# harskish/fluctus

Hardware: AMD Instinct MI355X
Metric: Mrays/s (primary+shadow) at 1080p, 8 bounces (higher is better)
Workload: dtype f32; 1 GPU; kitchen-proc (procedural stand-in for Country Kitchen OBJ), 1920x1080, 8 bounces, env-map MIS under night.hdr, separate material queues; width=1920, height=1080, max_bounces=8, triangles=495648, bvh=sbvh, bvh_nodes=342315, num_tasks_per_gpu=16777216, num_tasks_whole_job=16777216, scaling_mode=weak: --num-tasks paths in flight per rank, wavefronts_per_gpu=1, fused_logic_materials=True, fused_bsdf_set=1, ext_order=2, refill_extend=8208, overlap=2, regroup=1

## Files before the change

### fluctus_amd/csrc/api.hip

```cpp
#include "flx_ctx.h"
#include <cstring>
#include <cstdlib>

thread_local std::string flxd::g_create_error;

static uint32_t localPixels(const flx_ctx *c)
{
    uint32_t npix = c->params.width * c->params.height;
    if (npix <= c->fr.rank) return 1;
    return (npix - c->fr.rank + c->fr.nranks - 1) / c->fr.nranks;
}

static int allocMoments(flx_ctx *c)
{
    freeAll(c->momAllocs);
    c->fr.moments = nullptr;
    if (!c->moments || !c->fr.localPixels) return 0;
    const size_t n = (size_t)c->fr.localPixels * 4;
    HIPCHK(c, dalloc(c, c->momAllocs, &c->fr.moments, n) ? hipErrorOutOfMemory : hipSuccess);
    HIPCHK(c, hipMemsetAsync(c->fr.moments, 0, n * 4, c->stream));
    return 0;
}
static int allocAov(flx_ctx *c)
{
// ... 85 lines not shown
        if ((e = hipStreamCreateWithPriority(&c->stream2, hipStreamNonBlocking, pSecond)) != hipSuccess) return fail("hipStreamCreate", e);
    }
    if ((e = hipEventCreateWithFlags(&c->evPreExt, hipEventDisableTiming)) != hipSuccess || (e = hipEventCreateWithFlags(&c->evShadow, hipEventDisableTiming)) != hipSuccess ||
        (e = hipEventCreateWithFlags(&c->evPostLogic, hipEventDisableTiming)) != hipSuccess) return fail("hipEventCreate", e);
    const size_t N = num_tasks;
    c->st.numTasks = num_tasks;
    for (int r = 0; r < S_NUM_REC; r++) {
        if (dalloc(c, c->fixedAllocs, &c->st.rec[r], N)) return fail("hipMalloc(state)", hipErrorOutOfMemory);
        (void)hipMemsetAsync(c->st.rec[r], 0, N * sizeof(float4), c->stream);
    }
    if (dalloc(c, c->fixedAllocs, &c->st.phase, N) || dalloc(c, c->fixedAllocs, &c->mkStats, 4)) return fail("hipMalloc(state)", hipErrorOutOfMemory);
    (void)hipMemsetAsync(c->st.phase, 0, N * 4, c->stream); (void)hipMemsetAsync(c->mkStats, 0, 16, c->stream);
    if (dalloc(c, c->fixedAllocs, &c->st.blocked, N) || dalloc(c, c->fixedAllocs, &c->st.pickProb, N) || dalloc(c, c->fixedAllocs, &c->st.firstDiffuse, N))
        return fail("hipMalloc(state)", hipErrorOutOfMemory);
    (void)hipMemsetAsync(c->st.blocked, 0, N * 4, c->stream); (void)hipMemsetAsync(c->st.pickProb, 0, N * 4, c->stream); (void)hipMemsetAsync(c->st.firstDiffuse, 0, N * 4, c->stream);
    for (int q = 0; q < FLX_NUM_QUEUES; q++) {
        if (dalloc(c, c->fixedAllocs, &c->qs.q[q], N)) return fail("hipMalloc(queue)", hipErrorOutOfMemory);
        (void)hipMemsetAsync(c->qs.q[q], 0, N * 4, c->stream);
    }
    if (dalloc(c, c->fixedAllocs, &c->qs.counters, 8) || dalloc(c, c->fixedAllocs, &c->qs.cursors, FLX_NUM_BLOCK_CURSORS * FLX_CURSOR_STRIDE)) return fail("hipMalloc(counters)", hipErrorOutOfMemory);
    (void)hipMemsetAsync(c->qs.counters, 0, 32, c->stream);
    (void)hipMemsetAsync(c->qs.cursors, 0, 4 * FLX_NUM_BLOCK_CURSORS * FLX_CURSOR_STRIDE, c->stream);
    const size_t auxStride = logic_aux_stride(num_tasks);
    if (dalloc(c, c->fixedAllocs, &c->member, N) || dalloc(c, c->fixedAllocs, &c->blockCounts, (size_t)7 * auxStride) || dalloc(c, c->fixedAllocs, &c->blockOffsets, (size_t)7 * auxStride))
        return fail("hipMalloc(logic aux)", hipErrorOutOfMemory);
    if (dalloc(c, c->fixedAllocs, &c->logicError, 1)) return fail("hipMalloc(logic error flag)", hipErrorOutOfMemory);
    (void)hipMemsetAsync(c->logicError, 0, 4, c->stream);
    (void)hipMemsetAsync(c->blockCounts, 0, (size_t)7 * auxStride * 4, c->stream);
    (void)hipMemsetAsync(c->blockOffsets, 0, (size_t)7 * auxStride * 4, c->stream);
    { hipDeviceProp_t prop; if (hipGetDeviceProperties(&prop, device) == hipSuccess && prop.multiProcessorCount > 0) c->numCUs = prop.multiProcessorCount; }
    if (dalloc(c, c->fixedAllocs, &c->stats, FLX_NUM_TRACE_STATS)) return fail("hipMalloc(stats)", hipErrorOutOfMemory);
    (void)hipMemsetAsync(c->stats, 0, FLX_NUM_TRACE_STATS * 8, c->stream);
#ifdef FLX_LAB_RSTATS
    flxd::g_lab_rstats = c->stats;
#endif
    c->splitCapA = ((num_tasks / 2 / shadow_split_lists()) + 64u) & ~63u; c->splitCapB = ((num_tasks / 8 / shadow_split_lists()) + 64u) & ~63u;
    if (dalloc(c, c->fixedAllocs, &c->totals, 8)) return fail("hipMalloc(totals)", hipErrorOutOfMemory);
    (void)hipMemsetAsync(c->totals, 0, 64, c->stream);
    if (dalloc(c, c->fixedAllocs, &c->fr.currPixelIdx, 1)) return fail("hipMalloc(cursor)", hipErrorOutOfMemory);
    (void)hipMemsetAsync(c->fr.currPixelIdx, 0, 4, c->stream);
    c->fr.rank = 0; c->fr.nranks = 1; c->fr.localPixels = 0;
    if ((e = hipHostMalloc((void **)&c->pinned, sizeof(flx_queue_counters) * c->pinnedSlots)) != hipSuccess) return fail("hipHostMalloc", e);
    if ((e = hipHostMalloc((void **)&c->pinnedIdx, sizeof(uint32_t) * c->pinnedSlots)) != hipSuccess) return fail("hipHostMalloc", e);
    if ((e = hipHostMalloc((void **)&c->pinnedMk, 16 * c->pinnedSlots)) != hipSuccess) return fail("hipHostMalloc", e);
    {
        float4 *rgba; float2 *rec; float *pdf;
        if (dalloc(c, c->envAllocs, &rgba, 1) || dalloc(c, c->envAllocs, &rec, 1) || dalloc(c, c->envAllocs, &pdf, 1))
            return fail("hipMalloc(env)", hipErrorOutOfMemory);
        const float one = 1.0f; const float2 rec1 = make_float2(1.0f, 0.0f );
        (void)hipMemsetAsync(rgba, 0, 16, c->stream);
        (void)hipMemcpy(rec, &rec1, 8, hipMemcpyHostToDevice); (void)hipMemcpy(pdf, &one, 4, hipMemcpyHostToDevice);
        c->sc.envRGBA = rgba; c->sc.aliasRec = rec; c->sc.pdfTable = pdf; c->sc.envW = c->sc.envH = 1;
// ... 231 lines not shown
```

### fluctus_amd/csrc/api_wavefront.hip

```cpp
#include "flx_ctx.h"

struct Step { bool launchDeferred, commitRaw; int next; };
static Step transition(int ph, Call call)
{
    const bool deferred = ph == PH_DEFER_LOGIC || ph == PH_DEFER_LOGIC_RAYGEN;
    const bool chain = deferred || ph == PH_CHAIN || ph == PH_CHAIN_EXT;
    switch (call) {
    case CALL_LOGIC:     return {deferred, false, PH_IDLE};
    case CALL_RAYGEN:    if (ph == PH_DEFER_LOGIC) return {false, false, PH_DEFER_LOGIC_RAYGEN};
                         return {deferred, false, chain ? PH_CHAIN : PH_IDLE};
    case CALL_MATERIALS: if (deferred) return {false, false, PH_CHAIN};
                         return {false, true, chain ? PH_CHAIN : PH_IDLE};
    case CALL_EXTEND:    return {deferred, true, chain ? PH_CHAIN_EXT : PH_EXT};
    case CALL_SHADOW:    return {deferred, false, PH_IDLE};
    case CALL_QUIET:     return {deferred, false, deferred ? PH_CHAIN : ph};
    case CALL_NEUTRAL:   return {deferred, false, PH_IDLE};
    case CALL_PEEK:      return {deferred, true, deferred ? PH_CHAIN : ph};
    case CALL_OBSERVE:   return {deferred, true, PH_IDLE};
    }
    return {deferred, true, PH_IDLE};
}
void flxd::flushExt(flx_ctx *c) { if (c->qs.extPend) { launch_bump_extension(c->stream, c->qs.counters, c->qs.extPend); c->qs.extPend = 0; } }
static void flushExtIfPending(flx_ctx *c, uint32_t bits) { if (c->qs.extPend & bits) flushExt(c); }
static int runRaygen(flx_ctx *c, int appendExt = 1, bool alreadyDone = false, bool prepared = false)
// ... 12 lines not shown
    HIPCHK(c, hipSetDevice(c->device));
    launch_materialise(c->stream, c->st, c->sc, c->params, (uint32_t)c->numCUs);
    LAUNCHED(c);
    return 0;
}
static int extOrderFor(const flx_ctx *c, int fused, int raygenFirst) { return !fused ? 0 : (c->extOrder == 2 && (!raygenFirst || !c->raygenQueueEmpty)) ? 1 : c->extOrder; }
int flxd::fuseSetNow(const flx_ctx *c) { return c->params.wfSeparateQueues ? c->fuseSet : 31; }
static int runLogic(flx_ctx *c, int first, int fused, int raygenFirst)
{
    const int raw = (c->rawHits && fused != 0 && raygenFirst && !first) ? 1 : 0;
    if (!raw && materialise(c)) return 1;
    c->rawHits = false;
    flushExt(c);
#ifdef FLX_LAB_NOJOIN
    if (c->labIter >= 2) HIPCHK(c, hipStreamWaitEvent(c->stream, c->evLab[c->labIter & 1u], 0));
#endif
    const int order = extOrderFor(c, fused, raygenFirst);
    const int regen = (raw && c->regenOpt && c->lookback && logic_can_regenerate() && c->raygenQueueEmpty && c->fr.localPixels > 0 && c->numTasks <= (1u << 26)) ? 1 : 0;
    c->regenDone = regen != 0;
    if (regen) c->regenUsed = true;
    const int prep = (raw && !regen && c->prepOpt && c->raygenQueueEmpty && c->fr.localPixels > 0) ? 1 : 0;
    c->prepDone = prep != 0;
    if (++c->logicEpoch == 0u) c->logicEpoch = 1u;
    { ScopedTimer t(c, fused ? FLX_K_LOGIC_FUSED : FLX_K_LOGIC); launch_logic(c->stream, c->st, c->qs, c->sc, c->fr, c->params, c->member, c->blockCounts, c->blockOffsets, first, fused, raygenFirst, order, raw,
                                                                                c->lookback, c->logicEpoch, regen ? 1 : (prep ? 2 : 0), order == 2 ? 0 : 1, c->logicError, c->regroup,
                                                                                (!fused && c->ml.state.litWavefront()) ? &c->ml.t : nullptr); }
    LAUNCHED(c);
    c->matQueuesEmpty = false; c->raygenQueueEmpty = false;
    if (c->overlap == 2) HIPCHK(c, hipEventRecord(c->evPostLogic, c->stream));
    return 0;
}
static uint32_t materialBits(const flx_ctx *c)
{
    return c->params.wfSeparateQueues ? ((1u << FLX_Q_DIFFUSE) | (1u << FLX_Q_GLOSSY) | (1u << FLX_Q_GGX_REFL) | (1u << FLX_Q_GGX_REFR) | (1u << FLX_Q_DELTA)) : (1u << FLX_Q_DIFFUSE);
}
int flxd::enter(flx_ctx *c, Call call)
{
    const Step st = transition(c->phase, call);
    if (st.launchDeferred) {
        const bool withRaygen = c->phase == PH_DEFER_LOGIC_RAYGEN;
        c->phase = PH_CHAIN;
        HIPCHK(c, hipSetDevice(c->device));
        if (runLogic(c, c->pendFirst, 0, 0)) return 1;
        if (withRaygen && runRaygen(c)) return 1;
    }
    if (st.commitRaw && materialise(c)) return 1;
    c->phase = st.next;
    return 0;
// ... 141 lines not shown
```

### fluctus_amd/csrc/flx_ctx.h

```cpp
#pragma once
#include "flx_launch.h"
#include "flx_feature_state.h"
#include "../../include/fluctus_hip.h"
#include <string>
#include <vector>
#include <utility>
#include <rccl/rccl.h>

using namespace flxd;

namespace flxd {
struct PendingCounters { void *user; int slot; };
struct PendingEvent { int kernel; hipEvent_t a, b; };
inline void freeAll(std::vector<void *> &v) { for (void *p : v) (void)hipFree(p); v.clear(); }

enum Phase { PH_IDLE = 0, PH_DEFER_LOGIC = 1, PH_DEFER_LOGIC_RAYGEN = 2, PH_CHAIN = 3, PH_CHAIN_EXT = 4, PH_EXT = 5 };
enum Call {
    CALL_LOGIC, CALL_RAYGEN, CALL_MATERIALS, CALL_EXTEND, CALL_SHADOW,
    CALL_QUIET,
    CALL_NEUTRAL,
    CALL_PEEK,
    CALL_OBSERVE
};
}
// ... 6 lines not shown
#ifdef FLX_LAB_NOJOIN
    hipEvent_t evLab[2] = {nullptr, nullptr}; uint32_t labIter = 0; uint32_t *labCounters = nullptr;
#endif
    int phase = 0;
    int overlap = 2;
    int overlapOpt = -1;
    uint32_t *spill2 = nullptr;
    int fuse = 1;
    int extOrder = 0;
    int fuseSet = 1;
    int regroup = 0, regroupAuto = 0, regroupOpt = -1;
    int pendFirst = 0;
    bool matQueuesEmpty = false;
    bool raygenQueueEmpty = false;
    uint32_t numTasks = 0;
    std::string err;
    State st {};
    Queues qs {};
    Scene sc {};
    Frame fr {};
    flx_render_params params {};
    bool haveParams = false;
    uint32_t hostPixelIdx = 0;
    uint8_t *member = nullptr; uint32_t *blockCounts = nullptr, *blockOffsets = nullptr;
    unsigned long long *lookback = nullptr; uint32_t logicEpoch = 0; uint32_t *logicError = nullptr; int regenOpt = 0; bool regenDone = false; bool regenUsed = false; int prepOpt = 1; bool prepDone = false;
    uint32_t *spill = nullptr;
    unsigned long long *stats = nullptr;
    unsigned long long *totals = nullptr;
    uint32_t *mkStats = nullptr;
    uint32_t *pinnedMk = nullptr; std::vector<std::pair<void *, int>> pendingMk; int nextMkSlot = 0;
    bool statsOn = false;
    int xcdRemap = 0;
    int shadowTree = 4, extendTree = 4;
    int refillExt = 16 | (32 << 8), refillShadow = 0;
    int refillShadowOpt = -1;
    int shadowSplit = 0;
    uint32_t splitParity = 0;
    uint32_t splitLimit = 0;
    uint32_t *splitCounts = nullptr; uint4 *splitRecA = nullptr, *splitRecB = nullptr; uint32_t splitCapA = 0, splitCapB = 0;
    bool rawHits = false;
    bool cursorDirty[2] = {false, false};

    uint32_t wideInfo[8] = {0, 0, 0, 0, 0, 0, 0, 0};
    RefitTables rf;
    bool wideOK = false;
    uint32_t spillLevels = 0;
    int eagerBump = 0;
// ... 104 lines not shown
```

### fluctus_amd/csrc/flx_launch.h

```cpp
#pragma once
#include "flx_device.h"
#include <vector>

namespace flx { struct ad_params; struct rp_view; struct rp_params; }

namespace flxd {
struct RefitTables {
    uint32_t ntris = 0, nidx = 0, nmat = 0, nwtri = 0, nwleaf = 0;
    uint32_t *blevel = nullptr, *wlevel = nullptr;
    std::vector<uint32_t> blevelStart, wlevelStart;
    uint32_t *wtriOff = nullptr, *wleafOff = nullptr;
    float4 *wexact = nullptr;
    uint32_t *valid = nullptr;
    void *stage = nullptr;
    double *costSlab = nullptr;
    uint32_t *triStamp = nullptr, *bStamp = nullptr, *wStamp = nullptr, *lStamp = nullptr;
    size_t stampWords = 0;
    uint32_t epoch = 0;
    uint32_t *stageIdx = nullptr;
};
void launch_refit_validate(hipStream_t, const void *, const uint32_t *, uint32_t, const Scene &, const RefitTables &, uint32_t *);
void launch_refit(hipStream_t, const void *, const uint32_t *, uint32_t, const Scene &, const RefitTables &);
struct ObjectTables {
    uint32_t nobjects = 0, members = 0;
// ... 20 lines not shown
    *p0 = ld3(t[0]); *p1 = ld3(t[3]); *p2 = ld3(t[6]);
}
__device__ __forceinline__ int ml_material(const Scene &sc, uint32_t tri) { return sc.tris[tri].matId; }
template <bool MESH> struct MeshArg { static constexpr bool on = false; __device__ MeshLights get() const { return MeshLights(); } };
template <> struct MeshArg<true> { static constexpr bool on = true; MeshLights t; __device__ MeshLights get() const { return t; } };
uint32_t mesh_light_runs(uint32_t n);
void launch_mesh_light_build(hipStream_t, const Scene &, const MeshLights &);
void launch_mesh_light_probe(hipStream_t, const Scene &, const MeshLights &, const float *, uint32_t, uint32_t *, float *);
uint32_t pose_blocks(uint32_t members);
void launch_pose(hipStream_t, const ObjectTables &, uint32_t count);
void launch_object_of_triangle(hipStream_t, const ObjectTables &, uint32_t *objectOfTri);
void launch_block_scan(hipStream_t, uint32_t *blockCounts, uint32_t nb, uint32_t *total);
size_t tree_cost_slab_doubles(const RefitTables &);
double *launch_tree_cost(hipStream_t, const Scene &, const RefitTables &, double *);
void launch_extend(hipStream_t, const State &, const Queues &, const Scene &, const flx_render_params &, uint32_t *, unsigned long long *, int);
void launch_shadow(hipStream_t, const State &, const Queues &, const Scene &, const flx_render_params &, uint32_t *, unsigned long long *, int);
void launch_extend4(hipStream_t, const State &, const Queues &, const Scene &, const flx_render_params &, uint32_t *, unsigned long long *);
void launch_shadow4(hipStream_t, const State &, const Queues &, const Scene &, const flx_render_params &, uint32_t *, unsigned long long *);
void launch_shadow4_split(hipStream_t, const State &, const Queues &, const Scene &, const flx_render_params &, uint32_t *, uint32_t *, uint32_t, uint4 *, uint32_t, uint4 *, uint32_t, int, int, uint32_t);
uint32_t shadow_split_lists(); uint32_t shadow_split_count_words();
void launch_extend4r(hipStream_t, const State &, const Queues &, const Scene &, const flx_render_params &, uint32_t *, uint32_t, int, uint32_t *);
void launch_shadow4r(hipStream_t, const State &, const Queues &, const Scene &, const flx_render_params &, uint32_t *, uint32_t, int, uint32_t *);
void launch_logic(hipStream_t, const State &, const Queues &, const Scene &, const Frame &, const flx_render_params &, uint8_t *, uint32_t *, uint32_t *, int, int, int, int, int,
                  unsigned long long *, uint32_t, int, int, uint32_t *, int, const MeshLights *);
void launch_env_nee_table(hipStream_t, const Scene &, float4 *, uint32_t);
int logic_can_regenerate();
uint32_t logic_lookback_words(uint32_t numTasks);
void launch_materialise(hipStream_t, const State &, const Scene &, const flx_render_params &, uint32_t);
void launch_materials(hipStream_t, const State &, const Queues &, const Scene &, uint32_t);
void launch_materials_after_fused(hipStream_t, const State &, const Queues &, const Scene &, uint32_t, int);
uint32_t fused_queue_mask(int);
uint32_t logic_aux_stride(uint32_t);
void launch_reset(hipStream_t, const State &, const Queues &, const Frame &, const flx_render_params &);
void launch_raygen(hipStream_t, const State &, const Queues &, const Frame &, const flx_render_params &, int, int);
void launch_postprocess(hipStream_t, const Frame &, const flx_render_params &);
void launch_state_export(hipStream_t, const State &, float *, float);
void launch_state_import(hipStream_t, const State &, const float *);
void launch_math_probe(hipStream_t, int, const float *, const float *, uint32_t, uint32_t *);
void launch_mk_reset(hipStream_t, const State &, const Frame &, const flx_render_params &);
void launch_mk_raygen(hipStream_t, const State &, const flx_render_params &, const uint32_t *, uint32_t);
void launch_mk_next_vertex(hipStream_t, const State &, const Scene &, const Frame &, const flx_render_params &, uint32_t *, uint32_t *, const uint32_t *, uint32_t, const MeshLights *);
void launch_mk_sample_bsdf(hipStream_t, const State &, const Scene &, const Frame &, const flx_render_params &, uint32_t *, uint32_t *, const uint32_t *, uint32_t, const MeshLights *);
void launch_mk_splat(hipStream_t, const State &, const Frame &, const flx_render_params &, uint32_t *, int, const uint32_t *, uint32_t);
uint32_t adaptive_blocks(uint32_t);
void launch_adaptive_update(hipStream_t, const float4 *, int, int, const ad_params &, uint8_t *, uint32_t *, uint32_t *, uint32_t *);
void launch_end_iteration(hipStream_t, uint32_t *, unsigned long long *, uint32_t *, uint32_t, uint32_t, uint32_t *);
void launch_bump_extension(hipStream_t, uint32_t *, uint32_t);
void launch_deinterleave(hipStream_t, const float *, float *, uint32_t, uint32_t, uint32_t);
struct DnGuided; struct DnVg;
template <class F> void launch_denoise(hipStream_t, const Frame &, float4 *, float4 *, float4 *, float2 *, float *, int, int, int, float, float, float,
                                       float, const flx_render_params &);
void launch_gbuffer(hipStream_t, const Scene &, const flx_render_params &, uint32_t *, uint32_t, int, float4 *, uint32_t, uint32_t *, const uint32_t *);
void launch_reproject(hipStream_t, const rp_view &, const rp_params &, const float4 *, const float4 *, const float4 *, const float4 *, float4 *, float4 *);
void launch_reproject_motion(hipStream_t, const rp_view &, const rp_params &, const float4 *, const float4 *, const float4 *, const float4 *, float4 *, float4 *,
                             const uint32_t *, const uint32_t *, const float4 *, uint32_t);
// ... 5 lines not shown
```

### fluctus_amd/csrc/logic.hip

```cpp
#include "flx_bsdf.h"
#include "flx_trace.h"
#include "flx_denoise.h"
#include "flx_launch.h"
#include "flx_splat.h"
#include "flx_light.h"

namespace flxd {

#ifndef LOGIC_BLOCK
#define LOGIC_BLOCK 256
#endif
__host__ __device__ constexpr bool fuse_inlines_list(int fuse, uint32_t ml)
{
    return ml == 1u ? (fuse & USE_DIFFUSE) != 0 : ml == 2u ? (fuse & USE_GLOSSY) != 0 : ml == 3u ? (fuse & USE_GGX_REFL) != 0
         : ml == 4u ? (fuse & USE_GGX_REFR) != 0 : ml == 5u ? (fuse & USE_DELTA) != 0 : false;
}
#define NUM_LISTS 7

#ifndef LOGIC_FULL_STORES
#define LOGIC_FULL_STORES 1
#endif
#ifndef LOGIC_REGROUP
#define LOGIC_REGROUP 1
#endif
#ifndef LOGIC_LAZY_HITN
#define LOGIC_LAZY_HITN 1
#endif
#ifndef LOGIC_REGROUP_MIN_BLOCKS
#define LOGIC_REGROUP_MIN_BLOCKS 5
#endif

struct LogicAux {
    uint8_t *member;
    uint32_t *blockCounts;
    uint32_t *blockOffsets;
    uint32_t numBlocks;
    uint32_t stride;
    unsigned long long *lookback;
    uint32_t epoch;
    uint32_t regen;
    uint32_t appendExt;
    uint32_t *error;
};

#define LB_VALUE(x) ((uint32_t)((x) & 0x3FFFFFFull))
#define LB_FLAG(x) ((uint32_t)(((x) >> 26) & 3ull))
#define LB_EPOCH(x) ((uint32_t)((x) >> 28))
#define LB_PACK(e, f, v) (((unsigned long long)(e) << 28) | ((unsigned long long)(f) << 26) | (unsigned long long)(v))
__device__ __forceinline__ uint32_t wave_sum7(uint32_t v, bool take)
{
    uint32_t s = 0u;
    #pragma unroll
    for (int b = 0; b < 7; b++) s += (uint32_t)__popcll(__ballot(take && ((v >> b) & 1u))) << b;
    return s;
}
__device__ __forceinline__ uint32_t lookback_exclusive(const LogicAux &aux, uint32_t wave, uint32_t count)
{
    const uint32_t lane = lane_id();
    const uint32_t win = (uint32_t)__popcll(__ballot(true));
// ... 2 lines not shown
    if (wave == 0u) return 0u;
    uint32_t sum = 0u;
    long long j = (long long)wave - 1;
    for (uint32_t spins = 0;;) {
        const long long idx = j - (long long)lane;
        unsigned long long v = LB_PACK(aux.epoch, 2u, 0u);
        if (idx >= 0) v = __hip_atomic_load(st + idx, __ATOMIC_RELAXED, __HIP_MEMORY_SCOPE_AGENT);
        const bool ok = LB_EPOCH(v) == aux.epoch && LB_FLAG(v) != 0u;
        const uint64_t b2 = __ballot(ok && LB_FLAG(v) == 2u), bad = __ballot(!ok);
        const uint32_t first2 = b2 ? (uint32_t)__ffsll((long long)b2) - 1u : win;
        const uint64_t need = first2 >= 64u ? ~0ull : ((1ull << first2) | ((1ull << first2) - 1ull));
        if (bad & need) {
            if (++spins > (1u << 22)) { if (lane == 0u) *aux.error = 1u; break; }
            __builtin_amdgcn_s_sleep(2);
            continue;
        }
        sum += wave_sum7(LB_VALUE(v), lane < first2);
        if (b2) { sum += (uint32_t)__shfl((int)LB_VALUE(v), (int)first2, 64); break; }
        j -= (long long)win;
    }
    if (lane == 0u) __hip_atomic_store(st + wave, LB_PACK(aux.epoch, 2u, sum + count), __ATOMIC_RELAXED, __HIP_MEMORY_SCOPE_AGENT);
    return sum;
}

__device__ __forceinline__ uint32_t material_list(int type, uint32_t separate)
{
    if (!separate) return 1u;
    switch (type) {
    case FLX_BXDF_DIFFUSE: return 1u;
    case FLX_BXDF_GLOSSY: return 2u;
    case FLX_BXDF_GGX_ROUGH_REFLECTION: return 3u;
    case FLX_BXDF_GGX_ROUGH_DIELECTRIC: return 4u;
    case FLX_BXDF_IDEAL_REFLECTION:
    case FLX_BXDF_IDEAL_DIELECTRIC: return 5u;
    default: return 0u;
    }
}

#ifndef LOGIC_MIN_BLOCKS
#define LOGIC_MIN_BLOCKS 0
#endif
template <int FUSE, bool RAW = false, bool REGROUP = false, bool MESH = false>
__global__ __launch_bounds__(LOGIC_BLOCK, (REGROUP ? LOGIC_REGROUP_MIN_BLOCKS : LOGIC_MIN_BLOCKS) > 0 ? (REGROUP ? LOGIC_REGROUP_MIN_BLOCKS : LOGIC_MIN_BLOCKS) : 1) void k_logic(State st, Scene sc, Frame fr, flx_render_params p, LogicAux aux, Queues qs, uint32_t firstIteration, MeshArg<MESH> meshArg)
{
    const MeshLights mesh = meshArg.get();
    auto kinds = [&]() { return light_kind_probs(p.useEnvMap, p.useAreaLight, MESH && lamps_pickable(mesh)); };
// ... 374 lines not shown
            wr4(st.at(S_ORIG, gid), or4);
            wr4(st.at(S_DIR, gid), dr4);
            splat();
        }
    }

    if (gid < st.numTasks) aux.member[gid] = (uint8_t)member;

    __shared__ uint32_t s_cnt[NUM_LISTS][LOGIC_BLOCK / 64];
    const uint32_t wave = threadIdx.x >> 6;
    const uint32_t ml = member >> 2;
    uint64_t b0 = __ballot(member & 1u), b1 = __ballot(member & 2u);
    uint64_t m1 = __ballot(ml == 1u), m2 = __ballot(ml == 2u), m3 = __ballot(ml == 3u), m4 = __ballot(ml == 4u), m5 = __ballot(ml == 5u);
    if ((threadIdx.x & 63u) == 0u) {
        s_cnt[0][wave] = (uint32_t)__popcll(b0); s_cnt[1][wave] = (uint32_t)__popcll(b1);
        s_cnt[2][wave] = (uint32_t)__popcll(m1); s_cnt[3][wave] = (uint32_t)__popcll(m2);
        s_cnt[4][wave] = (uint32_t)__popcll(m3); s_cnt[5][wave] = (uint32_t)__popcll(m4); s_cnt[6][wave] = (uint32_t)__popcll(m5);
    }
    __syncthreads();
    if (threadIdx.x < NUM_LISTS) {
        uint32_t s = 0;
        for (int w = 0; w < LOGIC_BLOCK / 64; w++) s += s_cnt[threadIdx.x][w];
        aux.blockCounts[threadIdx.x * aux.stride + blockIdx.x] = s;
    }
}

__global__ __launch_bounds__(1024) void k_queue_scan(LogicAux aux, uint32_t *counters)
{
    __shared__ uint32_t s_wave[16];
    const uint32_t listToCounter[NUM_LISTS] = {FLX_Q_RAYGEN, FLX_Q_SHADOW, FLX_Q_DIFFUSE, FLX_Q_GLOSSY, FLX_Q_GGX_REFL, FLX_Q_GGX_REFR, FLX_Q_DELTA};
    const uint32_t nb = aux.numBlocks;
    const uint32_t per = ((nb + 1023u) / 1024u + 3u) & ~3u;
    const int l = blockIdx.x;
    const uint32_t *cnt = aux.blockCounts + (size_t)l * aux.stride;
    uint32_t *off = aux.blockOffsets + (size_t)l * aux.stride;
    const uint32_t base = counters[listToCounter[l]];
    const uint32_t lo = threadIdx.x * per;
    uint32_t s = 0;
    for (uint32_t i = 0; i < per; i += 4) {
        if (lo + i < nb) {
            const uint4 v = *reinterpret_cast<const uint4 *>(cnt + lo + i);
            s += v.x + v.y + v.z + v.w;
        }
    }
    const uint32_t lane = threadIdx.x & 63u, wave = threadIdx.x >> 6;
    uint32_t inc = s;
    for (int d = 1; d < 64; d <<= 1) { const uint32_t v = __shfl_up(inc, d, 64); if (lane >= (uint32_t)d) inc += v; }
    if (lane == 63u) s_wave[wave] = inc;
    __syncthreads();
    if (wave == 0u) {
        uint32_t w = lane < 16u ? s_wave[lane] : 0u, wi = w;
        for (int d = 1; d < 16; d <<= 1) { const uint32_t v = __shfl_up(wi, d, 64); if (lane >= (uint32_t)d) wi += v; }
        if (lane < 16u) s_wave[lane] = wi - w;
        if (lane == 15u) counters[listToCounter[l]] = base + wi;
    }
    __syncthreads();
    uint32_t run = base + s_wave[wave] + inc - s;
    for (uint32_t i = 0; i < per; i += 4) {
        if (lo + i < nb) {
            const uint4 v = *reinterpret_cast<const uint4 *>(cnt + lo + i);
            uint4 o;
            o.x = run; run += v.x; o.y = run; run += v.y; o.z = run; run += v.z; o.w = run; run += v.w;
            *reinterpret_cast<uint4 *>(off + lo + i) = o;
        }
    }
}

__global__ __launch_bounds__(LOGIC_BLOCK) void k_queue_scatter(Queues qs, LogicAux aux, uint32_t numTasks, int fuse, uint32_t raygenFirst, uint32_t byPathId)
{
    const uint32_t gid = blockIdx.x * LOGIC_BLOCK + threadIdx.x;
    const uint32_t member = gid < numTasks ? aux.member[gid] : 0u;
    const uint32_t ml = member >> 2;
    const uint32_t wave = threadIdx.x >> 6;
    __shared__ uint32_t s_cnt[NUM_LISTS][LOGIC_BLOCK / 64];
    __shared__ uint32_t s_off[NUM_LISTS];
    if (threadIdx.x < NUM_LISTS) s_off[threadIdx.x] = aux.blockOffsets[(size_t)threadIdx.x * aux.stride + blockIdx.x];
    uint64_t bal[NUM_LISTS];
    bal[0] = __ballot(member & 1u); bal[1] = __ballot(member & 2u);
    bal[2] = __ballot(ml == 1u); bal[3] = __ballot(ml == 2u); bal[4] = __ballot(ml == 3u); bal[5] = __ballot(ml == 4u); bal[6] = __ballot(ml == 5u);
    if ((threadIdx.x & 63u) == 0u)
        for (int l = 0; l < NUM_LISTS; l++) s_cnt[l][wave] = (uint32_t)__popcll(bal[l]);
    __syncthreads();
    uint32_t *const outq[NUM_LISTS] = {qs.q[FLX_Q_RAYGEN], qs.q[FLX_Q_SHADOW], qs.q[FLX_Q_DIFFUSE], qs.q[FLX_Q_GLOSSY], qs.q[FLX_Q_GGX_REFL], qs.q[FLX_Q_GGX_REFR], qs.q[FLX_Q_DELTA]};
    #pragma unroll
    for (int l = 0; l < NUM_LISTS; l++) {
        bool in = l == 0 ? (member & 1u) : l == 1 ? ((member & 2u) != 0u) : (ml == (uint32_t)(l - 1));
        if (in) {
            uint32_t r = s_off[l];
            for (uint32_t w = 0; w < wave; w++) r += s_cnt[l][w];
            r += mbcnt(bal[l]);
            outq[l][r] = gid;
            if (fuse != 0 && byPathId == 0u && l >= 2 && fuse_inlines_list(fuse, (uint32_t)(l - 1))) {
                uint32_t base = ext_len(qs) + (raygenFirst ? qs.counters[FLX_Q_RAYGEN] : 0u);
                for (int q = FLX_Q_DIFFUSE; q < FLX_Q_DIFFUSE + (l - 2); q++) base += qs.counters[q];
                qs.q[FLX_Q_EXTENSION][base + r] = gid;
            }
        }
    }
    if (fuse != 0 && byPathId == 1u && ml != 0u) {
        uint32_t r = s_off[2] + s_off[3] + s_off[4] + s_off[5] + s_off[6];
        for (uint32_t w = 0; w < wave; w++) r += s_cnt[2][w] + s_cnt[3][w] + s_cnt[4][w] + s_cnt[5][w] + s_cnt[6][w];
        r += mbcnt(bal[2] | bal[3] | bal[4] | bal[5] | bal[6]);
        qs.q[FLX_Q_EXTENSION][ext_len(qs) + (raygenFirst ? qs.counters[FLX_Q_RAYGEN] : 0u) + r] = gid;
    }
    if (fuse != 0 && byPathId == 2u && ((member & 1u) != 0u || ml != 0u)) {
        uint32_t r = s_off[0] + s_off[2] + s_off[3] + s_off[4] + s_off[5] + s_off[6];
        for (uint32_t w = 0; w < wave; w++) r += s_cnt[0][w] + s_cnt[2][w] + s_cnt[3][w] + s_cnt[4][w] + s_cnt[5][w] + s_cnt[6][w];
        r += mbcnt(bal[0] | bal[2] | bal[3] | bal[4] | bal[5] | bal[6]);
        qs.q[FLX_Q_EXTENSION][ext_len(qs) + r] = gid;
    }
}

uint32_t logic_aux_stride(uint32_t numTasks)
{
    const uint32_t blocks = (numTasks + LOGIC_BLOCK - 1) / LOGIC_BLOCK;
    const uint32_t per = ((blocks + 1023u) / 1024u + 3u) & ~3u;
    return per * 1024u;
}

uint32_t fused_queue_mask(int fuse)
{
    uint32_t m = 0;
    for (uint32_t ml = 1; ml <= 5; ml++) if (fuse_inlines_list(fuse, ml)) m |= 1u << (FLX_Q_DIFFUSE + ml - 1);
    return m;
}

void launch_logic(hipStream_t s, const State &st, const Queues &qs, const Scene &sc, const Frame &fr, const flx_render_params &p,
                  uint8_t *member, uint32_t *blockCounts, uint32_t *blockOffsets, int firstIteration, int fuse, int raygenFirst, int extByPathId, int raw,
                  unsigned long long *lookback, uint32_t epoch, int regen, int regenAppendExt, uint32_t *error, int regroup, const MeshLights *meshLights)
{
    uint32_t blocks = (st.numTasks + LOGIC_BLOCK - 1) / LOGIC_BLOCK;
    LogicAux aux{member, blockCounts, blockOffsets, blocks, logic_aux_stride(st.numTasks), lookback, epoch, (uint32_t)(raw ? regen : 0), (uint32_t)regenAppendExt, error};
    const bool rg = LOGIC_REGROUP && raw && regroup && fuse == USE_ALL && !firstIteration && st.numTasks % LOGIC_BLOCK == 0u;
    const dim3 g(blocks), b(LOGIC_BLOCK);
    switch (fuse) {
    case USE_DIFFUSE:
        if (raw) hipLaunchKernelGGL((k_logic<USE_DIFFUSE, true>), g, b, 0, s, st, sc, fr, p, aux, qs, (uint32_t)firstIteration, MeshArg<false>());
        else hipLaunchKernelGGL((k_logic<USE_DIFFUSE, false>), g, b, 0, s, st, sc, fr, p, aux, qs, (uint32_t)firstIteration, MeshArg<false>());
        break;
    case USE_ALL:
        if (rg) hipLaunchKernelGGL((k_logic<USE_ALL, true, true>), g, b, 0, s, st, sc, fr, p, aux, qs, (uint32_t)firstIteration, MeshArg<false>());
        else if (raw) hipLaunchKernelGGL((k_logic<USE_ALL, true>), g, b, 0, s, st, sc, fr, p, aux, qs, (uint32_t)firstIteration, MeshArg<false>());
        else hipLaunchKernelGGL((k_logic<USE_ALL, false>), g, b, 0, s, st, sc, fr, p, aux, qs, (uint32_t)firstIteration, MeshArg<false>());
        break;
    default:
        fuse = 0;
        if (meshLights) hipLaunchKernelGGL((k_logic<0, false, false, true>), g, b, 0, s, st, sc, fr, p, aux, qs, (uint32_t)firstIteration, MeshArg<true>{*meshLights});
        else hipLaunchKernelGGL(k_logic<0>, g, b, 0, s, st, sc, fr, p, aux, qs, (uint32_t)firstIteration, MeshArg<false>());
        break;
    }
    hipLaunchKernelGGL(k_queue_scan, dim3(NUM_LISTS), dim3(1024), 0, s, aux, qs.counters);
    hipLaunchKernelGGL(k_queue_scatter, g, b, 0, s, qs, aux, st.numTasks, fuse, (uint32_t)raygenFirst, (uint32_t)extByPathId);
}
int logic_can_regenerate() { return LOGIC_FULL_STORES != 0 ? 1 : 0; }
uint32_t logic_lookback_words(uint32_t numTasks) { return (numTasks + 63u) / 64u; }

}
```

Baseline: 6731 Mrays/s.

## Fuse queue scan and scatter into one segmented queue-build kernel

Replaces the two-kernel queue compaction (a 7-block global scan over per-block counts followed by a per-path scatter) with a single k_queue_build kernel. k_logic now atomically accumulates per-segment list totals and snapshots the queue counters. The build kernel derives segment bases from those totals, scans the block counts within each segment locally, and scatters four paths per lane using packed member bytes and vector stores. The goal is to drop a kernel launch and the serial 7-block scan, and to cut scatter memory traffic. The cost is added atomics in k_logic, double-buffered totals zeroed by parity, and redundant partial sums over all segments in every build block.

```diff
diff --git a/fluctus_amd/csrc/api.hip b/fluctus_amd/csrc/api.hip
--- a/fluctus_amd/csrc/api.hip
+++ b/fluctus_amd/csrc/api.hip
@@ -131,12 +131,13 @@
     (void)hipMemsetAsync(c->qs.counters, 0, 32, c->stream);
     (void)hipMemsetAsync(c->qs.cursors, 0, 4 * FLX_NUM_BLOCK_CURSORS * FLX_CURSOR_STRIDE, c->stream);
     const size_t auxStride = logic_aux_stride(num_tasks);
-    if (dalloc(c, c->fixedAllocs, &c->member, N) || dalloc(c, c->fixedAllocs, &c->blockCounts, (size_t)7 * auxStride) || dalloc(c, c->fixedAllocs, &c->blockOffsets, (size_t)7 * auxStride))
+    const size_t queueAuxWords = logic_queue_aux_words(num_tasks);
+    if (dalloc(c, c->fixedAllocs, &c->member, N) || dalloc(c, c->fixedAllocs, &c->blockCounts, (size_t)7 * auxStride) || dalloc(c, c->fixedAllocs, &c->queueAux, queueAuxWords))
         return fail("hipMalloc(logic aux)", hipErrorOutOfMemory);
     if (dalloc(c, c->fixedAllocs, &c->logicError, 1)) return fail("hipMalloc(logic error flag)", hipErrorOutOfMemory);
     (void)hipMemsetAsync(c->logicError, 0, 4, c->stream);
     (void)hipMemsetAsync(c->blockCounts, 0, (size_t)7 * auxStride * 4, c->stream);
-    (void)hipMemsetAsync(c->blockOffsets, 0, (size_t)7 * auxStride * 4, c->stream);
+    (void)hipMemsetAsync(c->queueAux, 0, queueAuxWords * 4, c->stream);
     { hipDeviceProp_t prop; if (hipGetDeviceProperties(&prop, device) == hipSuccess && prop.multiProcessorCount > 0) c->numCUs = prop.multiProcessorCount; }
     if (dalloc(c, c->fixedAllocs, &c->stats, FLX_NUM_TRACE_STATS)) return fail("hipMalloc(stats)", hipErrorOutOfMemory);
     (void)hipMemsetAsync(c->stats, 0, FLX_NUM_TRACE_STATS * 8, c->stream);
diff --git a/fluctus_amd/csrc/api_wavefront.hip b/fluctus_amd/csrc/api_wavefront.hip
--- a/fluctus_amd/csrc/api_wavefront.hip
+++ b/fluctus_amd/csrc/api_wavefront.hip
@@ -58,8 +58,9 @@
     const int prep = (raw && !regen && c->prepOpt && c->raygenQueueEmpty && c->fr.localPixels > 0) ? 1 : 0;
     c->prepDone = prep != 0;
     if (++c->logicEpoch == 0u) c->logicEpoch = 1u;
-    { ScopedTimer t(c, fused ? FLX_K_LOGIC_FUSED : FLX_K_LOGIC); launch_logic(c->stream, c->st, c->qs, c->sc, c->fr, c->params, c->member, c->blockCounts, c->blockOffsets, first, fused, raygenFirst, order, raw,
+    { ScopedTimer t(c, fused ? FLX_K_LOGIC_FUSED : FLX_K_LOGIC); launch_logic(c->stream, c->st, c->qs, c->sc, c->fr, c->params, c->member, c->blockCounts, c->queueAux, first, fused, raygenFirst, order, raw,
                                                                                 c->lookback, c->logicEpoch, regen ? 1 : (prep ? 2 : 0), order == 2 ? 0 : 1, c->logicError, c->regroup,
+                                                                                c->queueParity ^= 1u, (uint32_t)c->numCUs,
                                                                                 (!fused && c->ml.state.litWavefront()) ? &c->ml.t : nullptr); }
     LAUNCHED(c);
     c->matQueuesEmpty = false; c->raygenQueueEmpty = false;
diff --git a/fluctus_amd/csrc/flx_ctx.h b/fluctus_amd/csrc/flx_ctx.h
--- a/fluctus_amd/csrc/flx_ctx.h
+++ b/fluctus_amd/csrc/flx_ctx.h
@@ -52,7 +52,8 @@
     flx_render_params params {};
     bool haveParams = false;
     uint32_t hostPixelIdx = 0;
-    uint8_t *member = nullptr; uint32_t *blockCounts = nullptr, *blockOffsets = nullptr;
+    uint8_t *member = nullptr; uint32_t *blockCounts = nullptr;
+    uint32_t *queueAux = nullptr; uint32_t queueParity = 0;
     unsigned long long *lookback = nullptr; uint32_t logicEpoch = 0; uint32_t *logicError = nullptr; int regenOpt = 0; bool regenDone = false; bool regenUsed = false; int prepOpt = 1; bool prepDone = false;
     uint32_t *spill = nullptr;
     unsigned long long *stats = nullptr;
diff --git a/fluctus_amd/csrc/flx_launch.h b/fluctus_amd/csrc/flx_launch.h
--- a/fluctus_amd/csrc/flx_launch.h
+++ b/fluctus_amd/csrc/flx_launch.h
@@ -66,7 +66,7 @@
 void launch_extend4r(hipStream_t, const State &, const Queues &, const Scene &, const flx_render_params &, uint32_t *, uint32_t, int, uint32_t *);
 void launch_shadow4r(hipStream_t, const State &, const Queues &, const Scene &, const flx_render_params &, uint32_t *, uint32_t, int, uint32_t *);
 void launch_logic(hipStream_t, const State &, const Queues &, const Scene &, const Frame &, const flx_render_params &, uint8_t *, uint32_t *, uint32_t *, int, int, int, int, int,
-                  unsigned long long *, uint32_t, int, int, uint32_t *, int, const MeshLights *);
+                  unsigned long long *, uint32_t, int, int, uint32_t *, int, uint32_t, uint32_t, const MeshLights *);
 void launch_env_nee_table(hipStream_t, const Scene &, float4 *, uint32_t);
 int logic_can_regenerate();
 uint32_t logic_lookback_words(uint32_t numTasks);
@@ -75,6 +75,7 @@
 void launch_materials_after_fused(hipStream_t, const State &, const Queues &, const Scene &, uint32_t, int);
 uint32_t fused_queue_mask(int);
 uint32_t logic_aux_stride(uint32_t);
+uint32_t logic_queue_aux_words(uint32_t);
 void launch_reset(hipStream_t, const State &, const Queues &, const Frame &, const flx_render_params &);
 void launch_raygen(hipStream_t, const State &, const Queues &, const Frame &, const flx_render_params &, int, int);
 void launch_postprocess(hipStream_t, const Frame &, const flx_render_params &);
diff --git a/fluctus_amd/csrc/flx_queue_build.h b/fluctus_amd/csrc/flx_queue_build.h
--- /dev/null
+++ b/fluctus_amd/csrc/flx_queue_build.h
@@ -0,0 +1,89 @@
+#pragma once
+#include <stdint.h>
+
+#if defined(__HIPCC__) || defined(__CUDACC__)
+#define FLX_QB_HD __host__ __device__ inline
+#else
+#define FLX_QB_HD inline
+#endif
+
+namespace flxqb {
+
+enum : uint32_t {
+    QB_LISTS = 7u,
+    QB_BLOCK = 256u,
+    QB_SEG_BLOCKS = 64u,
+    QB_SEG_PATHS = QB_BLOCK * QB_SEG_BLOCKS,
+    QB_TILE = 256u,
+    QB_THREADS = 256u,
+    QB_WAVES = QB_THREADS / 64u,
+    QB_STEPS = QB_SEG_BLOCKS / QB_WAVES,
+    QB_MAX_PARTS = QB_STEPS
+};
+
+FLX_QB_HD uint32_t qb_blocks(uint32_t numTasks) { return (uint32_t)(((uint64_t)numTasks + QB_BLOCK - 1u) / QB_BLOCK); }
+FLX_QB_HD uint32_t qb_segments(uint32_t numTasks) { return (qb_blocks(numTasks) + QB_SEG_BLOCKS - 1u) / QB_SEG_BLOCKS; }
+FLX_QB_HD uint32_t qb_count_stride(uint32_t numTasks) { const uint32_t s = qb_segments(numTasks); return (s ? s : 1u) * QB_SEG_BLOCKS; }
+FLX_QB_HD uint32_t qb_totals_words(uint32_t numTasks) { const uint32_t s = qb_segments(numTasks); return QB_LISTS * (s ? s : 1u); }
+FLX_QB_HD uint32_t qb_aux_words(uint32_t numTasks) { return 2u * qb_totals_words(numTasks) + 8u; }
+FLX_QB_HD uint32_t qb_snapshot_at(uint32_t numTasks) { return 2u * qb_totals_words(numTasks); }
+
+FLX_QB_HD uint64_t qb_cap(uint32_t numCUs, uint32_t perCU) { return (uint64_t)(numCUs ? numCUs : 1u) * (perCU ? perCU : 1u); }
+FLX_QB_HD uint32_t qb_parts(uint32_t segments, uint32_t numCUs, uint32_t perCU)
+{
+    uint32_t parts = 1u;
+    while (parts < QB_MAX_PARTS && (uint64_t)segments * (2u * parts) <= qb_cap(numCUs, perCU)) parts *= 2u;
+    return parts;
+}
+FLX_QB_HD uint32_t qb_grid(uint32_t segments, uint32_t numCUs, uint32_t perCU)
+{
+    const uint64_t cap = qb_cap(numCUs, perCU), units = (uint64_t)segments * qb_parts(segments, numCUs, perCU);
+    const uint32_t g = units < cap ? (uint32_t)units : (uint32_t)cap;
+    return g ? g : 1u;
+}
+FLX_QB_HD uint32_t qb_share(uint32_t segments, uint32_t grid) { return (segments + grid - 1u) / grid; }
+FLX_QB_HD void qb_owned(uint32_t block, uint32_t grid, uint32_t segments, uint32_t parts, uint32_t *first, uint32_t *end)
+{
+    const uint64_t share = parts > 1u ? 1u : qb_share(segments, grid);
+    const uint64_t f = parts > 1u ? block / parts : share * block, e = f + share;
+    *first = f < segments ? (uint32_t)f : segments;
+    *end = e < segments ? (uint32_t)e : segments;
+}
+FLX_QB_HD void qb_tiles(uint32_t block, uint32_t parts, uint32_t *tile0, uint32_t *steps)
+{
+    *tile0 = (block % parts) * (QB_SEG_BLOCKS / parts);
+    *steps = QB_STEPS / parts;
+}
+
+FLX_QB_HD void qb_partial(const uint32_t *totals, uint32_t segments, uint32_t first, uint32_t t, uint32_t n, uint32_t *before, uint32_t *all)
+{
+    uint32_t b = 0u, a = 0u;
+    for (uint32_t s = t; s < segments; s += n) { const uint32_t v = totals[s]; a += v; if (s < first) b += v; }
+    *before = b; *all = a;
+}
+
+FLX_QB_HD uint32_t qb_in_list(uint32_t byte, uint32_t list)
+{
+    return list == 0u ? (byte & 1u) : list == 1u ? ((byte >> 1) & 1u) : (((byte >> 2) & 7u) == list - 1u ? 1u : 0u);
+}
+FLX_QB_HD uint32_t qb_bits(uint32_t word, uint32_t list)
+{
+    return qb_in_list(word & 0xFFu, list) | (qb_in_list((word >> 8) & 0xFFu, list) << 1) | (qb_in_list((word >> 16) & 0xFFu, list) << 2) | (qb_in_list(word >> 24, list) << 3);
+}
+FLX_QB_HD uint32_t qb_bits_material(uint32_t word)
+{
+    const uint32_t m = word & 0x1C1C1C1Cu;
+    const uint32_t any = (m | (m >> 1) | (m >> 2)) & 0x04040404u;
+    return ((any >> 2) | (any >> 9) | (any >> 16) | (any >> 23)) & 0xFu;
+}
+FLX_QB_HD uint32_t qb_bits_traced(uint32_t word)
+{
+    const uint32_t r = word & 0x01010101u;
+    return (qb_bits_material(word) | r | (r >> 7) | (r >> 14) | (r >> 21)) & 0xFu;
+}
+FLX_QB_HD uint32_t qb_count4(uint32_t bits) { return (bits & 1u) + ((bits >> 1) & 1u) + ((bits >> 2) & 1u) + ((bits >> 3) & 1u); }
+FLX_QB_HD uint32_t qb_rank4(uint32_t bits, uint32_t k) { return qb_count4(bits & ((1u << k) - 1u)); }
+FLX_QB_HD uint64_t qb_first_path(uint32_t seg, uint32_t tile, uint32_t lane) { return ((uint64_t)seg * QB_SEG_BLOCKS + tile) * QB_TILE + 4u * lane; }
+FLX_QB_HD uint32_t qb_valid(uint64_t p, uint32_t numTasks) { return p >= numTasks ? 0u : numTasks - p >= 4u ? 4u : (uint32_t)(numTasks - p); }
+
+}
diff --git a/fluctus_amd/csrc/logic.hip b/fluctus_amd/csrc/logic.hip
--- a/fluctus_amd/csrc/logic.hip
+++ b/fluctus_amd/csrc/logic.hip
@@ -4,6 +4,7 @@
 #include "flx_launch.h"
 #include "flx_splat.h"
 #include "flx_light.h"
+#include "flx_queue_build.h"
 
 namespace flxd {
 
@@ -33,8 +34,10 @@
 struct LogicAux {
     uint8_t *member;
     uint32_t *blockCounts;
-    uint32_t *blockOffsets;
+    uint32_t *segTotals;
+    uint32_t *snapshot;
     uint32_t numBlocks;
+    uint32_t numSegs;
     uint32_t stride;
     unsigned long long *lookback;
     uint32_t epoch;
@@ -83,6 +86,10 @@
     if (lane == 0u) __hip_atomic_store(st + wave, LB_PACK(aux.epoch, 2u, sum + count), __ATOMIC_RELAXED, __HIP_MEMORY_SCOPE_AGENT);
     return sum;
 }
+
+static_assert(LOGIC_BLOCK == flxqb::QB_BLOCK && NUM_LISTS == flxqb::QB_LISTS, "flx_queue_build.h counts in k_logic's blocks and lists");
+__host__ __device__ constexpr uint32_t list_counter(uint32_t l) { return l == 0u ? (uint32_t)FLX_Q_RAYGEN : l + 1u; }
+static_assert(list_counter(1) == FLX_Q_SHADOW && list_counter(2) == FLX_Q_DIFFUSE && list_counter(6) == FLX_Q_DELTA, "queue numbering");
 
 __device__ __forceinline__ uint32_t material_list(int type, uint32_t separate)
 {
@@ -503,101 +510,116 @@
         uint32_t s = 0;
         for (int w = 0; w < LOGIC_BLOCK / 64; w++) s += s_cnt[threadIdx.x][w];
         aux.blockCounts[threadIdx.x * aux.stride + blockIdx.x] = s;
-    }
-}
-
-__global__ __launch_bounds__(1024) void k_queue_scan(LogicAux aux, uint32_t *counters)
-{
-    __shared__ uint32_t s_wave[16];
-    const uint32_t listToCounter[NUM_LISTS] = {FLX_Q_RAYGEN, FLX_Q_SHADOW, FLX_Q_DIFFUSE, FLX_Q_GLOSSY, FLX_Q_GGX_REFL, FLX_Q_GGX_REFR, FLX_Q_DELTA};
-    const uint32_t nb = aux.numBlocks;
-    const uint32_t per = ((nb + 1023u) / 1024u + 3u) & ~3u;
-    const int l = blockIdx.x;
-    const uint32_t *cnt = aux.blockCounts + (size_t)l * aux.stride;
-    uint32_t *off = aux.blockOffsets + (size_t)l * aux.stride;
-    const uint32_t base = counters[listToCounter[l]];
-    const uint32_t lo = threadIdx.x * per;
-    uint32_t s = 0;
-    for (uint32_t i = 0; i < per; i += 4) {
-        if (lo + i < nb) {
-            const uint4 v = *reinterpret_cast<const uint4 *>(cnt + lo + i);
-            s += v.x + v.y + v.z + v.w;
-        }
-    }
+        if (s != 0u) atomicAdd(aux.segTotals + threadIdx.x * aux.numSegs + blockIdx.x / flxqb::QB_SEG_BLOCKS, s);
+        if (blockIdx.x == 0u) aux.snapshot[threadIdx.x] = qs.counters[list_counter(threadIdx.x)];
+    }
+}
+
+#ifndef QUEUE_BUILD_BLOCKS_PER_CU
+#define QUEUE_BUILD_BLOCKS_PER_CU 4
+#endif
+struct QueueBuild {
+    const uint8_t *member; const uint32_t *blockCounts; const uint32_t *totals; uint32_t *zero; const uint32_t *snapshot;
+    uint32_t stride, numTasks, numSegs, totalsWords;
+    uint32_t parts;
+    int fuse; uint32_t raygenFirst, byPathId;
+};
+__device__ __forceinline__ uint32_t wave_sum(uint32_t v) { for (int d = 32; d > 0; d >>= 1) v += __shfl_xor(v, d, 64); return v; }
+__device__ __forceinline__ uint32_t prefix_of_count4(uint32_t n) { return mbcnt(__ballot(n & 1u)) + 2u * mbcnt(__ballot(n & 2u)) + 4u * mbcnt(__ballot(n & 4u)); }
+__device__ __forceinline__ void emit4(uint32_t *q, uint32_t slot, uint32_t bits, uint32_t gid)
+{
+    if (bits == 0xFu && (slot & 3u) == 0u) { *reinterpret_cast<uint4 *>(q + slot) = make_uint4(gid, gid + 1u, gid + 2u, gid + 3u); return; }
+    if (bits & 1u) q[slot++] = gid;
+    if (bits & 2u) q[slot++] = gid + 1u;
+    if (bits & 4u) q[slot++] = gid + 2u;
+    if (bits & 8u) q[slot] = gid + 3u;
+}
+__device__ __forceinline__ uint32_t load_member4(const uint8_t *member, uint64_t p, uint32_t numTasks)
+{
+    const uint32_t valid = flxqb::qb_valid(p, numTasks);
+    if (valid == 4u) return *reinterpret_cast<const uint32_t *>(member + p);
+    uint32_t w = 0u;
+    for (uint32_t k = 0; k < valid; k++) w |= (uint32_t)member[p + k] << (8u * k);
+    return w;
+}
+
+__global__ __launch_bounds__(flxqb::QB_THREADS) void k_queue_build(Queues qs, QueueBuild a)
+{
+    using namespace flxqb;
+    __shared__ uint32_t s_base[NUM_LISTS];
+    __shared__ uint32_t s_new[NUM_LISTS];
+    __shared__ uint32_t s_off[NUM_LISTS][QB_SEG_BLOCKS];
     const uint32_t lane = threadIdx.x & 63u, wave = threadIdx.x >> 6;
-    uint32_t inc = s;
-    for (int d = 1; d < 64; d <<= 1) { const uint32_t v = __shfl_up(inc, d, 64); if (lane >= (uint32_t)d) inc += v; }
-    if (lane == 63u) s_wave[wave] = inc;
+    uint32_t seg0, seg1;
+    qb_owned(blockIdx.x, gridDim.x, a.numSegs, a.parts, &seg0, &seg1);
+    uint32_t tile0, steps;
+    qb_tiles(blockIdx.x, a.parts, &tile0, &steps);
+    for (uint32_t i = blockIdx.x * QB_THREADS + threadIdx.x; i < a.totalsWords; i += gridDim.x * QB_THREADS) a.zero[i] = 0u;
+    for (uint32_t l = wave; l < NUM_LISTS; l += QB_WAVES) {
+        uint32_t before, all;
+        qb_partial(a.totals + (size_t)l * a.numSegs, a.numSegs, seg0, lane, 64u, &before, &all);
+        before = wave_sum(before); all = wave_sum(all);
+        if (lane == 0u) { const uint32_t snap = a.snapshot[l]; s_base[l] = snap + before; s_new[l] = snap + all; }
+    }
     __syncthreads();
-    if (wave == 0u) {
-        uint32_t w = lane < 16u ? s_wave[lane] : 0u, wi = w;
-        for (int d = 1; d < 16; d <<= 1) { const uint32_t v = __shfl_up(wi, d, 64); if (lane >= (uint32_t)d) wi += v; }
-        if (lane < 16u) s_wave[lane] = wi - w;
-        if (lane == 15u) counters[listToCounter[l]] = base + wi;
-    }
-    __syncthreads();
-    uint32_t run = base + s_wave[wave] + inc - s;
-    for (uint32_t i = 0; i < per; i += 4) {
-        if (lo + i < nb) {
-            const uint4 v = *reinterpret_cast<const uint4 *>(cnt + lo + i);
-            uint4 o;
-            o.x = run; run += v.x; o.y = run; run += v.y; o.z = run; run += v.z; o.w = run; run += v.w;
-            *reinterpret_cast<uint4 *>(off + lo + i) = o;
-        }
-    }
-}
-
-__global__ __launch_bounds__(LOGIC_BLOCK) void k_queue_scatter(Queues qs, LogicAux aux, uint32_t numTasks, int fuse, uint32_t raygenFirst, uint32_t byPathId)
-{
-    const uint32_t gid = blockIdx.x * LOGIC_BLOCK + threadIdx.x;
-    const uint32_t member = gid < numTasks ? aux.member[gid] : 0u;
-    const uint32_t ml = member >> 2;
-    const uint32_t wave = threadIdx.x >> 6;
-    __shared__ uint32_t s_cnt[NUM_LISTS][LOGIC_BLOCK / 64];
-    __shared__ uint32_t s_off[NUM_LISTS];
-    if (threadIdx.x < NUM_LISTS) s_off[threadIdx.x] = aux.blockOffsets[(size_t)threadIdx.x * aux.stride + blockIdx.x];
-    uint64_t bal[NUM_LISTS];
-    bal[0] = __ballot(member & 1u); bal[1] = __ballot(member & 2u);
-    bal[2] = __ballot(ml == 1u); bal[3] = __ballot(ml == 2u); bal[4] = __ballot(ml == 3u); bal[5] = __ballot(ml == 4u); bal[6] = __ballot(ml == 5u);
-    if ((threadIdx.x & 63u) == 0u)
-        for (int l = 0; l < NUM_LISTS; l++) s_cnt[l][wave] = (uint32_t)__popcll(bal[l]);
-    __syncthreads();
+    if (blockIdx.x == 0u && threadIdx.x < NUM_LISTS) qs.counters[list_counter(threadIdx.x)] = s_new[threadIdx.x];
+    if (seg0 == seg1) return;
+    uint32_t extBase = qs.counters[FLX_Q_EXTENSION];
+    if (qs.extPend) for (uint32_t l = 0; l < NUM_LISTS; l++) if (qs.extPend & (1u << list_counter(l))) extBase += s_new[l];
+    if (a.byPathId != 2u && a.raygenFirst) extBase += s_new[0];
     uint32_t *const outq[NUM_LISTS] = {qs.q[FLX_Q_RAYGEN], qs.q[FLX_Q_SHADOW], qs.q[FLX_Q_DIFFUSE], qs.q[FLX_Q_GLOSSY], qs.q[FLX_Q_GGX_REFL], qs.q[FLX_Q_GGX_REFR], qs.q[FLX_Q_DELTA]};
-    #pragma unroll
-    for (int l = 0; l < NUM_LISTS; l++) {
-        bool in = l == 0 ? (member & 1u) : l == 1 ? ((member & 2u) != 0u) : (ml == (uint32_t)(l - 1));
-        if (in) {
-            uint32_t r = s_off[l];
-            for (uint32_t w = 0; w < wave; w++) r += s_cnt[l][w];
-            r += mbcnt(bal[l]);
-            outq[l][r] = gid;
-            if (fuse != 0 && byPathId == 0u && l >= 2 && fuse_inlines_list(fuse, (uint32_t)(l - 1))) {
-                uint32_t base = ext_len(qs) + (raygenFirst ? qs.counters[FLX_Q_RAYGEN] : 0u);
-                for (int q = FLX_Q_DIFFUSE; q < FLX_Q_DIFFUSE + (l - 2); q++) base += qs.counters[q];
-                qs.q[FLX_Q_EXTENSION][base + r] = gid;
-            }
-        }
-    }
-    if (fuse != 0 && byPathId == 1u && ml != 0u) {
-        uint32_t r = s_off[2] + s_off[3] + s_off[4] + s_off[5] + s_off[6];
-        for (uint32_t w = 0; w < wave; w++) r += s_cnt[2][w] + s_cnt[3][w] + s_cnt[4][w] + s_cnt[5][w] + s_cnt[6][w];
-        r += mbcnt(bal[2] | bal[3] | bal[4] | bal[5] | bal[6]);
-        qs.q[FLX_Q_EXTENSION][ext_len(qs) + (raygenFirst ? qs.counters[FLX_Q_RAYGEN] : 0u) + r] = gid;
-    }
-    if (fuse != 0 && byPathId == 2u && ((member & 1u) != 0u || ml != 0u)) {
-        uint32_t r = s_off[0] + s_off[2] + s_off[3] + s_off[4] + s_off[5] + s_off[6];
-        for (uint32_t w = 0; w < wave; w++) r += s_cnt[0][w] + s_cnt[2][w] + s_cnt[3][w] + s_cnt[4][w] + s_cnt[5][w] + s_cnt[6][w];
-        r += mbcnt(bal[0] | bal[2] | bal[3] | bal[4] | bal[5] | bal[6]);
-        qs.q[FLX_Q_EXTENSION][ext_len(qs) + r] = gid;
-    }
-}
-
-uint32_t logic_aux_stride(uint32_t numTasks)
-{
-    const uint32_t blocks = (numTasks + LOGIC_BLOCK - 1) / LOGIC_BLOCK;
-    const uint32_t per = ((blocks + 1023u) / 1024u + 3u) & ~3u;
-    return per * 1024u;
-}
+    uint32_t *const ext = qs.q[FLX_Q_EXTENSION];
+
+    for (uint32_t seg = seg0; seg < seg1; seg++) {
+        uint32_t mw[QB_STEPS];
+        #pragma unroll
+        for (uint32_t i = 0; i < QB_STEPS; i++) mw[i] = i < steps ? load_member4(a.member, qb_first_path(seg, tile0 + wave + QB_WAVES * i, lane), a.numTasks) : 0u;
+        if (seg != seg0) __syncthreads();
+        for (uint32_t l = wave; l < NUM_LISTS; l += QB_WAVES) {
+            const uint32_t c = a.blockCounts[(size_t)l * a.stride + (size_t)seg * QB_SEG_BLOCKS + lane];
+            uint32_t inc = c;
+            for (int d = 1; d < 64; d <<= 1) { const uint32_t v = __shfl_up(inc, d, 64); if (lane >= (uint32_t)d) inc += v; }
+            const uint32_t base = s_base[l];
+            s_off[l][lane] = base + inc - c;
+            if (lane == 63u) s_base[l] = base + inc;
+        }
+        __syncthreads();
+        #pragma unroll
+        for (uint32_t i = 0; i < QB_STEPS; i++) {
+            if (i >= steps) break;
+            const uint32_t tile = tile0 + wave + QB_WAVES * i;
+            const uint32_t w = mw[i];
+            const uint32_t gid = (uint32_t)qb_first_path(seg, tile, lane);
+            if (__ballot(w != 0u) == 0ull) continue;
+            uint32_t matOff = 0u;
+            #pragma unroll
+            for (int l = 0; l < NUM_LISTS; l++) {
+                const uint32_t off = s_off[l][tile];
+                if (l >= 2) matOff += off;
+                const uint32_t bits = qb_bits(w, (uint32_t)l);
+                if (__ballot(bits != 0u) == 0ull) continue;
+                const uint32_t r = off + prefix_of_count4(qb_count4(bits));
+                emit4(outq[l], r, bits, gid);
+                if (a.fuse != 0 && a.byPathId == 0u && l >= 2 && fuse_inlines_list(a.fuse, (uint32_t)(l - 1))) {
+                    uint32_t segBase = extBase;
+                    for (int m = 2; m < l; m++) segBase += s_new[m];
+                    emit4(ext, segBase + r, bits, gid);
+                }
+            }
+            if (a.fuse != 0 && a.byPathId == 1u) {
+                const uint32_t bits = qb_bits_material(w);
+                emit4(ext, extBase + matOff + prefix_of_count4(qb_count4(bits)), bits, gid);
+            }
+            if (a.fuse != 0 && a.byPathId == 2u) {
+                const uint32_t bits = qb_bits_traced(w);
+                emit4(ext, extBase + s_off[0][tile] + matOff + prefix_of_count4(qb_count4(bits)), bits, gid);
+            }
+        }
+    }
+}
+
+uint32_t logic_aux_stride(uint32_t numTasks) { return flxqb::qb_count_stride(numTasks); }
+uint32_t logic_queue_aux_words(uint32_t numTasks) { return flxqb::qb_aux_words(numTasks); }
 
 uint32_t fused_queue_mask(int fuse)
 {
@@ -607,11 +629,16 @@
 }
 
 void launch_logic(hipStream_t s, const State &st, const Queues &qs, const Scene &sc, const Frame &fr, const flx_render_params &p,
-                  uint8_t *member, uint32_t *blockCounts, uint32_t *blockOffsets, int firstIteration, int fuse, int raygenFirst, int extByPathId, int raw,
-                  unsigned long long *lookback, uint32_t epoch, int regen, int regenAppendExt, uint32_t *error, int regroup, const MeshLights *meshLights)
+                  uint8_t *member, uint32_t *blockCounts, uint32_t *queueAux, int firstIteration, int fuse, int raygenFirst, int extByPathId, int raw,
+                  unsigned long long *lookback, uint32_t epoch, int regen, int regenAppendExt, uint32_t *error, int regroup, uint32_t parity, uint32_t numCUs,
+                  const MeshLights *meshLights)
 {
     uint32_t blocks = (st.numTasks + LOGIC_BLOCK - 1) / LOGIC_BLOCK;
-    LogicAux aux{member, blockCounts, blockOffsets, blocks, logic_aux_stride(st.numTasks), lookback, epoch, (uint32_t)(raw ? regen : 0), (uint32_t)regenAppendExt, error};
+    const uint32_t tw = flxqb::qb_totals_words(st.numTasks);
+    parity &= 1u;
+    uint32_t *const totals = queueAux + (size_t)parity * tw;
+    LogicAux aux{member, blockCounts, totals, queueAux + flxqb::qb_snapshot_at(st.numTasks), blocks, flxqb::qb_segments(st.numTasks), logic_aux_stride(st.numTasks),
+                 lookback, epoch, (uint32_t)(raw ? regen : 0), (uint32_t)regenAppendExt, error};
     const bool rg = LOGIC_REGROUP && raw && regroup && fuse == USE_ALL && !firstIteration && st.numTasks % LOGIC_BLOCK == 0u;
     const dim3 g(blocks), b(LOGIC_BLOCK);
     switch (fuse) {
@@ -630,8 +657,8 @@
         else hipLaunchKernelGGL(k_logic<0>, g, b, 0, s, st, sc, fr, p, aux, qs, (uint32_t)firstIteration, MeshArg<false>());
         break;
     }
-    hipLaunchKernelGGL(k_queue_scan, dim3(NUM_LISTS), dim3(1024), 0, s, aux, qs.counters);
-    hipLaunchKernelGGL(k_queue_scatter, g, b, 0, s, qs, aux, st.numTasks, fuse, (uint32_t)raygenFirst, (uint32_t)extByPathId);
+    const QueueBuild qb{member, blockCounts, totals, queueAux + (size_t)(parity ^ 1u) * tw, aux.snapshot, aux.stride, st.numTasks, aux.numSegs, tw, flxqb::qb_parts(aux.numSegs, numCUs, QUEUE_BUILD_BLOCKS_PER_CU), fuse, (uint32_t)raygenFirst, (uint32_t)extByPathId};
+    hipLaunchKernelGGL(k_queue_build, dim3(flxqb::qb_grid(aux.numSegs, numCUs, QUEUE_BUILD_BLOCKS_PER_CU)), dim3(flxqb::QB_THREADS), 0, s, qs, qb);
 }
 int logic_can_regenerate() { return LOGIC_FULL_STORES != 0 ? 1 : 0; }
 uint32_t logic_lookback_words(uint32_t numTasks) { return (numTasks + 63u) / 64u; }
```

After: 6824 Mrays/s (median of 6 runs). 1.4% higher.
